# Gabrielcb/DaliID

Measured on AMD Instinct MI355X. Metric: images/sec (train step), higher is better.
Workload: dtype bf16; 1 GPU; configs[1]: ResNet-50 ReID bf16 256x128, PK batch 16x16=256 per GPU, center+proxy heads, Adam, EMA; global_batch=256, per_gpu_batch=256, parallelism=dp1

## Files before the change

daliid_amd/csrc/bnlin.hip:

```cpp
#include "kernels.h"
#include "reduce_finish.h"
#include <algorithm>

namespace dali {

namespace {
constexpr int BL_CH = 8;

__device__ __forceinline__ double block_sum_d(double v, double* red) {
    const int lane = threadIdx.x & 63, w = threadIdx.x >> 6;
#pragma unroll
    for (int o = 32; o > 0; o >>= 1) v += __shfl_xor(v, o, 64);
    __syncthreads();
    if (lane == 0) red[w] = v;
    __syncthreads();
    return (red[0] + red[1]) + (red[2] + red[3]);
}
__device__ __forceinline__ float ld_f(const float* p) { return *p; }
__device__ __forceinline__ float ld_f(const uint16_t* p) { return bf16_bits_to_f32(*p); }
}

constexpr int BL_SAV_MAX = 2048;
struct BnlinFin {
    const float* m2; double count; const float* gamma; const float* beta; float* running_mean; float* running_var; float momentum, eps;
// ... 359 lines not shown
    hipLaunchKernelGGL(bnlin_row_kernel, dim3(C / BL_CH), dim3(256), (size_t)(3 * BL_CH + 1) * w * sizeof(float), st, W, ut, m2, s_dz, C, w,
                       count, scale, mean, invstd, dW, dgamma, dbeta, wd1, ld1, qk);
    DALI_LAUNCH_CHECK();
#define BL_BWD(DEPTH) hipLaunchKernelGGL((bnlin_nt_gemm_kernel<uint16_t, true, true, false, DEPTH>), dim3(w / 32, w / 32), dim3(256), 0, st, Wt, C, Wt, C, qk, C, (float*)nullptr, wd2, ld2, \
                                         (const uint16_t*)nullptr, 0, (float*)nullptr, 0, qk + C, bvec)
    switch (C <= BL_SAV_MAX ? bnlin_depth(C) : 1) { case 8: BL_BWD(8); break; case 4: BL_BWD(4); break; case 2: BL_BWD(2); break; default: BL_BWD(1); }
#undef BL_BWD
    DALI_LAUNCH_CHECK();
    return DALI_OK;
}

}

using namespace dali;

static GatherGeom bl_geom(int P, int Ck) {
    GatherGeom g{};
    g.Hout = 1; g.Wout = P; g.Hin = 1; g.Win = P; g.Ck = Ck; g.R = 1; g.S = 1; g.stride = 1; g.pad = 0; g.mode = 0;
    g.pix_pitch = Ck; g.row_pitch = P * Ck; g.img_pitch = (long long)P * Ck; g.lw = g.lhw = -1;
    return g;
}

extern "C" int dali_bnlin_fwd(dali_ctx* ctx, void* stream, const uint16_t* a, const uint16_t* W, int P, int C, int w, const float* gamma,
                              const float* beta, float* running_mean, float* running_var, float momentum, float eps, float* gram, float* m2,
                              float* ut, float* scale, float* shift, float* mean, float* invstd) {
    DALI_REQUIRE(ctx && a && W && gamma && beta && gram && m2 && ut && scale && shift && mean && invstd, "dali_bnlin_fwd: null argument");
    DALI_REQUIRE(P > 0 && C % 32 == 0 && w % 32 == 0, "dali_bnlin_fwd: C %% 32, w %% 32 (C=%d w=%d)", C, w);
    hipStream_t st = (hipStream_t)stream;
    WGradArgs wa{};
    wa.dY = a; wa.X = a; wa.Cm = w; wa.P = P; wa.Ntot = w; wa.g = bl_geom(P, w);
    size_t wsb;
    wgrad_plan(w, w, P, 512, &wa.splits, &wa.pix_per_split, &wsb, 1, 0);
    const bool fused_cs = wgrad_colsum_supported(w, w, 1, P);
    const int cs_rows = wgrad_colsum_rows(w, w, 1, P, wa.splits);
    const size_t b_cs = align_up(std::max(colsum_partial_floats(P, w), (size_t)cs_rows * w) * 4, 256), b_sc = align_up(reduce_scratch_bytes(w, 1), 256);
    const size_t b_wt = align_up((size_t)C * w * 2, 256), b_dot = align_up((size_t)(w / 32) * C * 12, 256);
    char* ws = static_cast<char*>(workspace(ctx, align_up(wsb, 256) + b_cs + b_sc + b_wt + b_dot));
    if (!ws) return DALI_ERR_NOMEM;
    wa.partial = reinterpret_cast<float*>(ws);
    char* p = ws + align_up(wsb, 256);
    float* cs_partial = reinterpret_cast<float*>(p); p += b_cs;
    double* scratch = reinterpret_cast<double*>(p); p += b_sc;
    uint16_t* wt = reinterpret_cast<uint16_t*>(p); p += b_wt;
    float* dot = reinterpret_cast<float*>(p);
    int rc;
    if (fused_cs) wa.colsum = cs_partial;
    if ((rc = launch_igemm_wgrad(st, wa, gram, 0, fused_cs ? m2 : nullptr, cs_rows))) return rc;
    if (!fused_cs && (rc = launch_colsum(st, a, P, w, m2, cs_partial, scratch))) return rc;
    if ((rc = launch_weight_transpose(st, W, C, 1, w, wt))) return rc;
    return launch_bnlin_stats(st, W, wt, gram, m2, C, w, (double)P, gamma, beta, running_mean, running_var, momentum, eps, ut, dot, scale, shift, mean, invstd);
}

extern "C" int dali_bnlin_bwd(dali_ctx* ctx, void* stream, const uint16_t* dz, const uint16_t* a, const uint16_t* W, int P, int C, int w,
                              const float* ut, const float* m2, const float* scale, const float* mean, const float* invstd, float* dW,
                              float* dgamma, float* dbeta, uint16_t* wd1, uint16_t* wd2, float* bvec) {
    DALI_REQUIRE(ctx && dz && a && W && ut && m2 && scale && mean && invstd && dW && dgamma && dbeta && wd1 && wd2 && bvec, "dali_bnlin_bwd: null argument");
    DALI_REQUIRE(P > 0 && C % 32 == 0 && w % 32 == 0, "dali_bnlin_bwd: C %% 32, w %% 32 (C=%d w=%d)", C, w);
    hipStream_t st = (hipStream_t)stream;
    WGradArgs wa{};
    wa.dY = dz; wa.X = a; wa.Cm = C; wa.P = P; wa.Ntot = w; wa.g = bl_geom(P, w);
    size_t wsb;
    wgrad_plan(C, w, P, 512, &wa.splits, &wa.pix_per_split, &wsb, 1, 0);
    const bool fused_cs = wgrad_colsum_supported(C, w, 1, P);
    const int cs_rows = wgrad_colsum_rows(C, w, 1, P, wa.splits);
    const size_t b_cs = align_up(std::max(colsum_partial_floats(P, C), (size_t)cs_rows * C) * 4, 256), b_sc = align_up(reduce_scratch_bytes(C, 1), 256);
    const size_t b_v = align_up((size_t)C * 4, 256), b_wt = align_up((size_t)C * w * 2, 256);
    char* ws = static_cast<char*>(workspace(ctx, align_up(wsb, 256) + b_cs + b_sc + 3 * b_v + b_wt));
    if (!ws) return DALI_ERR_NOMEM;
    wa.partial = reinterpret_cast<float*>(ws);
    char* p = ws + align_up(wsb, 256);
    float* cs_partial = reinterpret_cast<float*>(p); p += b_cs;
    double* scratch = reinterpret_cast<double*>(p); p += b_sc;
    float* sdz = reinterpret_cast<float*>(p); p += b_v;
    float* qk = reinterpret_cast<float*>(p); p += 2 * b_v;
    uint16_t* wt = reinterpret_cast<uint16_t*>(p);
// ... 8 lines not shown
```

daliid_amd/csrc/conv.hip:

```cpp
#include "gemm_tile.h"
#include "kernels.h"
#include <cstdlib>
#include <type_traits>
#include <vector>
#include <string>
#include <cstdio>

namespace dali {

__device__ __forceinline__ void decode_pixel(const GatherGeom& g, int p, int& n, int& ho, int& wo) {
    if (g.lhw >= 0 && g.lw >= 0) {
        n = p >> g.lhw;
        const int rem = p & ((1 << g.lhw) - 1);
        ho = rem >> g.lw;
        wo = rem & ((1 << g.lw) - 1);
    } else {
        const int hw = g.Hout * g.Wout;
        n = p / hw;
        const int rem = p - n * hw;
        ho = rem / g.Wout;
        wo = rem - ho * g.Wout;
    }
}

// ... 1295 lines not shown
                const bf16x8_t fb = *reinterpret_cast<const bf16x8_t*>(patch + (boff[j] ^ (uint32_t)(h << 5)));
#pragma unroll
                for (int i = 0; i < FM; ++i) acc[i][j] = __builtin_amdgcn_mfma_f32_16x16x32_bf16(fa[i], fb, acc[i][j], 0, 0, 0);
            }
        }
        asm volatile("s_waitcnt lgkmcnt(0)" ::: "memory");
        __builtin_amdgcn_s_barrier();
    }
    conv_epilogue_g<TM, TN, FM, FN, 4, NT, (EPI == 3 || EPI == 5) ? EPI : 2>(a, acc, 0, tn, smem, 0, wn);
}

}
#include "fused1x1.h"
namespace dali {

__device__ __forceinline__ int wg_swz(int row) { return (row & 3) | (((row >> 3) & 1) << 2); }

typedef short s16x4_t __attribute__((ext_vector_type(4)));

__device__ __forceinline__ bf16x8_t tr_frag(const uint16_t* tile, int chunk32, int lane) {
    const int g = lane >> 4, q = (lane & 15) >> 2, p = lane & 3;
    const int row0 = 8 * g + q, row1 = row0 + 4;
    const int off0 = row0 * 128 + ((chunk32 ^ wg_swz(row0)) << 4) + 4 * p;
    const int off1 = row1 * 128 + ((chunk32 ^ wg_swz(row1)) << 4) + 4 * p;
    typedef __attribute__((address_space(3))) s16x4_t* lds_ptr_t;
    const s16x4_t a = __builtin_amdgcn_ds_read_tr16_b64_v4i16((lds_ptr_t)(tile + off0));
    const s16x4_t b = __builtin_amdgcn_ds_read_tr16_b64_v4i16((lds_ptr_t)(tile + off1));
    typedef short s16x8_t __attribute__((ext_vector_type(8)));
    const s16x8_t v = {a[0], a[1], a[2], a[3], b[0], b[1], b[2], b[3]};
    return __builtin_bit_cast(bf16x8_t, v);
}

struct TrPair { s16x4_t lo, hi; };
__device__ __forceinline__ s16x4_t ds_read_tr_raw(const uint16_t* p) {
    typedef __attribute__((address_space(3))) const uint16_t* lds_cptr_t;
    const uint32_t addr = (uint32_t)(uintptr_t)(lds_cptr_t)p;
    s16x4_t v;
    asm volatile("ds_read_b64_tr_b16 %0, %1" : "=v"(v) : "v"(addr));
    return v;
}
__device__ __forceinline__ TrPair tr_frag_raw(const uint16_t* tile, int chunk32, int lane) {
    const int g = lane >> 4, q = (lane & 15) >> 2, p = lane & 3;
    const int row0 = 8 * g + q, row1 = row0 + 4;
    const int off0 = row0 * 128 + ((chunk32 ^ wg_swz(row0)) << 4) + 4 * p;
    const int off1 = row1 * 128 + ((chunk32 ^ wg_swz(row1)) << 4) + 4 * p;
    return TrPair{ds_read_tr_raw(tile + off0), ds_read_tr_raw(tile + off1)};
}
__device__ __forceinline__ bf16x8_t tr_join(const TrPair& t) {
    typedef short s16x8_t __attribute__((ext_vector_type(8)));
    const s16x8_t v = {t.lo[0], t.lo[1], t.lo[2], t.lo[3], t.hi[0], t.hi[1], t.hi[2], t.hi[3]};
    return __builtin_bit_cast(bf16x8_t, v);
}
template <int N>
__device__ __forceinline__ void tr_settle(TrPair& a, TrPair& b, TrPair& c, TrPair& d) {
    static_assert(N == 0 || N == 8 || N == 10 || N == 16 || N == 18, "lgkmcnt immediates used by the callers");
    if constexpr (N == 0) asm volatile("s_waitcnt lgkmcnt(0)" : "+v"(a.lo), "+v"(a.hi), "+v"(b.lo), "+v"(b.hi), "+v"(c.lo), "+v"(c.hi), "+v"(d.lo), "+v"(d.hi));
    else if constexpr (N == 8) asm volatile("s_waitcnt lgkmcnt(8)" : "+v"(a.lo), "+v"(a.hi), "+v"(b.lo), "+v"(b.hi), "+v"(c.lo), "+v"(c.hi), "+v"(d.lo), "+v"(d.hi));
    else if constexpr (N == 10) asm volatile("s_waitcnt lgkmcnt(10)" : "+v"(a.lo), "+v"(a.hi), "+v"(b.lo), "+v"(b.hi), "+v"(c.lo), "+v"(c.hi), "+v"(d.lo), "+v"(d.hi));
    else if constexpr (N == 16) asm volatile("s_waitcnt lgkmcnt(15)" : "+v"(a.lo), "+v"(a.hi), "+v"(b.lo), "+v"(b.hi), "+v"(c.lo), "+v"(c.hi), "+v"(d.lo), "+v"(d.hi));
    else asm volatile("s_waitcnt lgkmcnt(15)" : "+v"(a.lo), "+v"(a.hi), "+v"(b.lo), "+v"(b.hi), "+v"(c.lo), "+v"(c.hi), "+v"(d.lo), "+v"(d.hi));
}

__device__ __forceinline__ void tr_settle_all(TrPair& a) { asm volatile("s_waitcnt lgkmcnt(0)" : "+v"(a.lo), "+v"(a.hi)); }

template <int FM, int FN>
__device__ __forceinline__ void store_slab_tiles(float* slab, const f32x4_t (&acc)[FM][FN], int m_first, int n_first, int Cm, int Ntot, int lane) {
    const int mr = m_first + (lane >> 4) * 4, nc = n_first + (lane & 15);
    if (m_first + 16 * FM <= Cm && n_first + 16 * FN <= Ntot) {
        float* row = slab + (size_t)mr * Ntot + nc;
#pragma unroll
        for (int i = 0; i < FM; ++i)
#pragma unroll
            for (int rr = 0; rr < 4; ++rr) {
                float* p = row + (size_t)(i * 16 + rr) * Ntot;
#pragma unroll
                for (int j = 0; j < FN; ++j) p[j * 16] = acc[i][j][rr];
            }
        return;
    }
#pragma unroll
    for (int i = 0; i < FM; ++i)
#pragma unroll
        for (int j = 0; j < FN; ++j) {
            const int n = nc + j * 16;
#pragma unroll
            for (int rr = 0; rr < 4; ++rr) {
                const int m = mr + i * 16 + rr;
                if (m < Cm && n < Ntot) slab[(size_t)m * Ntot + n] = acc[i][j][rr];
            }
        }
}

template <bool IN_BN>
__global__ __launch_bounds__(256) void igemm_wgrad_kernel(WGradArgs a, int tiles_m, int tiles_n) {
    constexpr int TILE = 32 * 128;
    __shared__ __attribute__((aligned(16))) uint16_t smem[2 * 2 * TILE];
    const int tid = threadIdx.x, lane = tid & 63, wave = tid >> 6;
    const int wm = wave >> 1, wn = wave & 1;
    const int tiles = tiles_m * tiles_n;
    const int tile = blockIdx.x % tiles, ks = blockIdx.x / tiles;
    const int tm = tile / tiles_n, tn = tile - tm * tiles_n;
    const int m0 = tm * 128, n0 = tn * 128;
    const GatherGeom g = a.g;

    const int c16 = tid & 15;
    const int am = m0 + c16 * 8;
// ... 1530 lines not shown
```

daliid_amd/csrc/kernels.h:

```cpp
#pragma once
#include "common.h"

namespace dali {

struct GatherGeom {
    int Hout, Wout;
    int Hin, Win;
    int Ck;
    int R, S, stride, pad;
    int mode;
    long long img_pitch;
    int row_pitch, pix_pitch;
    int lw, lhw;
    int sub, oph, opw, Hfull, Wfull;
    int r0, rstep, nr, s0, sstep, ns;
    int class_grid;
};

struct IGemmArgs {
    const uint16_t* W;
    const uint16_t* X;
    uint16_t* O;
    const uint16_t* Res;
    const uint8_t* res_mask;
// ... 45 lines not shown
void wgrad_plan(int Cm, int Ntot, int P, int target_blocks, int* splits, int* pix_per_split, size_t* ws_bytes, int taps = 1, int halo_w = 0);
int launch_igemm_wgrad(hipStream_t st, const WGradArgs& a, float* out, int accumulate, float* colsum_out = nullptr, int colsum_rows = 0);
int launch_splitk_reduce2(hipStream_t st, const float* partial, float* out, size_t elems, int splits, int accumulate,
                          const float* partial2, float* out2, size_t elems2, int splits2);
bool wgrad_colsum_supported(int Cm, int Ntot, int taps, int P);
int launch_splitk_reduce(hipStream_t st, const float* partial, float* out, size_t elems, int splits, int accumulate);

int launch_linear_fwd(hipStream_t st, const uint16_t* x, const uint16_t* w, const float* bias, int act, const uint16_t* residual, uint16_t* y,
                      uint16_t* pre, const uint16_t* dact_pre, int rows, int K, int N, const float* row_scale = nullptr);
int launch_linear_wgrad(hipStream_t st, const uint16_t* x, const uint16_t* dy, float* dw, int rows, int K, int N, float* slab,
                        float* dbias = nullptr, float* cs_partial = nullptr, bool* bias_done = nullptr);
size_t linear_wgrad_colsum_floats(int rows, int K, int N);
int wgrad_colsum_rows(int Cm, int Ntot, int taps, int P, int splits);
size_t linear_wgrad_slab_bytes(int rows, int K, int N);

int launch_bnlin_stats(hipStream_t st, const uint16_t* W, const uint16_t* Wt, const float* gram, const float* m2, int C, int w, double count, const float* gamma,
                       const float* beta, float* rm, float* rv, float momentum, float eps, float* ut, float* dot, float* scale, float* shift,
                       float* mean, float* invstd);
int launch_bnlin_ut(hipStream_t st, const uint16_t* W, const float* gram, int C, int w, float* ut);
int launch_bnlin_bwd(hipStream_t st, const uint16_t* W, const uint16_t* Wt, const float* ut, const float* m2, const float* s_dz, int C,
                     int w, double count, const float* scale, const float* mean, const float* invstd, float* dW, float* dgamma, float* dbeta,
                     uint16_t* wd1, uint16_t* wd2, float* bvec, float* qk, int ld1 = 0, int ld2 = 0);

constexpr int REDUCE_SMAX = 64;
inline size_t reduce_scratch_bytes(int C, int NV) { return (size_t)REDUCE_SMAX * C * NV * sizeof(double); }
int launch_bn_finalize(hipStream_t st, const float* partial, int tiles, int C, double count, const float* gamma, const float* beta,
                       float* rm, float* rv, float momentum, float eps, float* scale, float* shift, float* mean, float* invstd,
                       double* scratch);
int launch_bn_eval_coeffs(hipStream_t st, const float* gamma, const float* beta, const float* rm, const float* rv, float eps, int C,
                          float* scale, float* shift);
// ... 64 lines not shown
```

daliid_amd/csrc/resnet_plan.hip:

```cpp
#include "kernels.h"
#include <cstdio>
#include <cstring>
#include <new>
#include <string>
#include <vector>

using namespace dali;

namespace {

struct TensorInfo { std::string name; int64_t offset, numel; int shape[4]; int ndim; };

struct Conv {
    int cin, cout, r, s, stride, pad, hin, win, hout, wout;
    int64_t w_off;
    uint16_t* w_bf16;
    uint16_t* wt_bf16;
};
struct Bn {
    int C;
    int64_t g_off, b_off;
    int64_t rm_off, rv_off;
    float *scale, *shift, *mean, *invstd, *coef;
};
// ... 190 lines not shown
        int sp, pps; size_t wsb;
        wgrad_plan(wb, 224, (int)N * net->stem_h * net->stem_w, 512, &sp, &pps, &wsb, 7);
        max_slab = wsb;
    }
    for (auto& b : net->blocks) {
        const size_t pin = N * b.hin * b.win, pout = N * b.hout * b.wout;
        reserve(net, a, b.raw1, pin * b.width * 2);
        reserve(net, a, b.a1, pin * b.width * 2);
        reserve(net, a, b.raw2, pout * b.width * 2);
        reserve(net, a, b.a2, pout * b.width * 2);
        reserve(net, a, b.gram, (size_t)b.width * b.width * 4); reserve(net, a, b.m2, (size_t)b.width * 4);
        reserve(net, a, b.sdz, (size_t)b.cout * 4); reserve(net, a, b.bvec, (size_t)b.width * 4); reserve(net, a, b.qk, (size_t)b.cout * 8);
        reserve(net, a, b.wd1, (size_t)b.width * (b.cout + b.width) * 2);
        reserve(net, a, b.ut, (size_t)b.width * b.cout * 4); reserve(net, a, b.dot, (size_t)(b.width / 32) * b.cout * 12);
        max_cs = std::max(max_cs, std::max(colsum_partial_floats((int)pout, b.cout), colsum_partial_floats((int)pout, b.width)) * 4);
        int sp, pps; size_t wsb;
        wgrad_plan(b.width, b.width, (int)pout, 512, &sp, &pps, &wsb, 1, 0);
        max_slab = std::max(max_slab, wsb);
        max_cs = std::max(max_cs, (size_t)wgrad_colsum_rows(b.width, b.width, 1, (int)pout, sp) * b.width * 4);
        wgrad_plan(b.cout, b.width, (int)pout, 512, &sp, &pps, &wsb, 1, 0);
        max_cs = std::max(max_cs, (size_t)wgrad_colsum_rows(b.cout, b.width, 1, (int)pout, sp) * b.cout * 4);
        reserve(net, a, b.y, pout * b.cout * 2);
        reserve(net, a, b.ybits, pout * b.cout / 8);
        if (b.has_ds) reserve(net, a, b.rawd, pout * b.cout * 2);
        if (b.lin_ds) {
            reserve(net, a, b.gram_d, (size_t)b.cin * b.cin * 4); reserve(net, a, b.m2_d, (size_t)b.cin * 4);
            reserve(net, a, b.ut_d, (size_t)b.cin * b.cout * 4); reserve(net, a, b.bvec_d, (size_t)b.cin * 4); reserve(net, a, b.qk_d, (size_t)b.cout * 8);
            reserve(net, a, b.wdd, (size_t)b.cin * (b.cout + b.cin) * 2);
            int sp, pps; size_t wsb;
            wgrad_plan(b.cin, b.cin, (int)pin, 512, &sp, &pps, &wsb, 1, 0);
            max_slab = std::max(max_slab, wsb);
            max_cs = std::max(max_cs, std::max(colsum_partial_floats((int)pin, b.cin), (size_t)wgrad_colsum_rows(b.cin, b.cin, 1, (int)pin, sp) * b.cin) * 4);
        }
        b.cat_eval = b.has_ds && b.cd.stride == 1 && conv_cat_act_supported(b.cout, b.width, b.cin, (int)pout, 2);
        if (b.cat_eval) { reserve(net, a, b.wcat, (size_t)b.cout * 2 * (b.width + b.cin) * 2); reserve(net, a, b.shcat, (size_t)b.cout * 4); }
        reserve_bn(net, a, b.b1); reserve_bn(net, a, b.b2); reserve_bn(net, a, b.b3);
        if (b.has_ds) reserve_bn(net, a, b.bd);
        Conv* cs[4] = {&b.c1, &b.c2, &b.c3, b.has_ds ? &b.cd : nullptr};
        for (Conv* c : cs) {
            if (!c) continue;
            reserve(net, a, c->wt_bf16, (size_t)c->cin * c->r * c->s * c->cout * 2);
            const int P = (int)N * c->hout * c->wout;
            max_stat = std::max(max_stat, (size_t)igemm_conv_stat_tiles(c->cout, P, c->r * c->s * c->cin) * c->cout * 2 * 4);
            int sp, pps; size_t wsb;
            wgrad_plan(c->cout, c->r * c->s * c->cin, P, 512, &sp, &pps, &wsb, c->r * c->s, conv_halo_w(*c));
            max_slab = std::max(max_slab, wsb);
            max_act = std::max(max_act, (size_t)P * c->cout * 2);
// ... 186 lines not shown
    const uint16_t* x = net->pool0;
    for (auto& b : net->blocks) {
        b.x = const_cast<uint16_t*>(x);
        const size_t e1 = (size_t)net->N * b.hin * b.win * b.width, e2 = (size_t)net->N * b.hout * b.wout * b.width;
        if (!tr) {
            if ((rc = conv_bn_relu_eval(net, st, b.c1, b.b1, x, b.a1))) return rc;
            if ((rc = conv_bn_relu_eval(net, st, b.c2, b.b2, b.a1, b.a2))) return rc;
        } else {
            if ((rc = conv_bn_fwd(net, st, b.c1, b.b1, x, nullptr, b.raw1, tr))) return rc;
            if ((rc = launch_bn_act(st, b.raw1, b.b1.scale, b.b1.shift, nullptr, nullptr, nullptr, nullptr, 1, e1, b.width, b.a1, nullptr))) return rc;
            if ((rc = conv_bn_fwd(net, st, b.c2, b.b2, b.a1, nullptr, b.raw2, tr))) return rc;
            if ((rc = launch_bn_act(st, b.raw2, b.b2.scale, b.b2.shift, nullptr, nullptr, nullptr, nullptr, 1, e2, b.width, b.a2, nullptr))) return rc;
        }
        const int Pout = net->N * b.hout * b.wout;
        if (tr) {
            const Conv sq = square_conv(b.c3);
            WGradArgs wa{};
            wa.dY = b.a2; wa.X = b.a2; wa.partial = net->wgrad_slab; wa.Cm = b.width; wa.P = Pout; wa.Ntot = b.width;
            wa.g = conv_geom(sq, 0);
            size_t wsb;
            wgrad_plan(wa.Cm, wa.Ntot, wa.P, 512, &wa.splits, &wa.pix_per_split, &wsb, 1, 0);
            const bool fused_cs = wgrad_colsum_supported(wa.Cm, wa.Ntot, 1, wa.P);
            if (fused_cs) wa.colsum = net->cs_partial;
            if ((rc = launch_igemm_wgrad(st, wa, b.gram, 0, fused_cs ? b.m2 : nullptr, fused_cs ? wgrad_colsum_rows(wa.Cm, wa.Ntot, 1, wa.P, wa.splits) : 0))) return rc;
            if (!fused_cs && (rc = launch_colsum(st, b.a2, Pout, b.width, b.m2, net->cs_partial, net->red_scratch))) return rc;
            if ((rc = launch_bnlin_stats(st, b.c3.w_bf16, b.c3.wt_bf16, b.gram, b.m2, b.cout, b.width, (double)Pout, net->P + b.b3.g_off, net->P + b.b3.b_off,
                                         net->B + b.b3.rm_off, net->B + b.b3.rv_off, 0.1f, 1e-5f, b.ut, b.dot, b.b3.scale, b.b3.shift, b.b3.mean,
                                         b.b3.invstd))) return rc;
        }
        if (!tr && b.cat_eval) {
            if ((rc = launch_fold_cat_weights(st, net->P + b.c3.w_off, net->P + b.cd.w_off, b.b3.scale, b.bd.scale, b.b3.shift, b.bd.shift, b.cout, b.width,
                                              b.cin, 2, b.wcat, b.shcat))) return rc;
            IGemmArgs ca{};
            ca.W = b.wcat; ca.X = b.a2; ca.X2 = x; ca.Ck1 = b.width; ca.x_rep = 2; ca.O = b.y; ca.out_shift = b.shcat; ca.out_relu = 1;
            ca.Cm = b.cout; ca.P = Pout;
            Conv cat = b.c3;
            cat.cin = 2 * (b.width + b.cin);
            ca.g = conv_geom(cat, 0);
            if ((rc = launch_igemm_conv(st, ca))) return rc;
            x = b.y;
            continue;
        }
        IGemmArgs a{};
        a.W = b.c3.w_bf16; a.X = b.a2; a.O = b.y; a.Res = x; a.out_scale = b.b3.scale; a.out_shift = b.b3.shift; a.out_relu = 1;
        if (b.has_ds) {
            if ((rc = conv_bn_fwd(net, st, b.cd, b.bd, x, nullptr, b.rawd, tr))) return rc;
            a.Res = b.rawd; a.res_scale = b.bd.scale; a.bias = b.bd.shift;
            if (b.lin_ds && tr) {
                Conv sq = b.cd;
                sq.cout = b.cd.cin;
                WGradArgs wa{};
                wa.dY = x; wa.X = x; wa.partial = net->wgrad_slab; wa.Cm = b.cin; wa.P = Pout; wa.Ntot = b.cin;
                wa.g = conv_geom(sq, 0);
                size_t wsb;
                wgrad_plan(wa.Cm, wa.Ntot, wa.P, 512, &wa.splits, &wa.pix_per_split, &wsb, 1, 0);
                const bool fused_cs = wgrad_colsum_supported(wa.Cm, wa.Ntot, 1, wa.P);
                if (fused_cs) wa.colsum = net->cs_partial;
                if ((rc = launch_igemm_wgrad(st, wa, b.gram_d, 0, fused_cs ? b.m2_d : nullptr, fused_cs ? wgrad_colsum_rows(wa.Cm, wa.Ntot, 1, wa.P, wa.splits) : 0))) return rc;
                if (!fused_cs && (rc = launch_colsum(st, x, Pout, b.cin, b.m2_d, net->cs_partial, net->red_scratch))) return rc;
                if ((rc = launch_bnlin_ut(st, b.cd.w_bf16, b.gram_d, b.cout, b.cin, b.ut_d))) return rc;
            }
        }
        a.bits_out = tr ? b.ybits : nullptr;
        a.Cm = b.cout; a.P = Pout; a.g = conv_geom(b.c3, 0);
        if ((rc = launch_igemm_conv(st, a))) return rc;
        x = b.y;
    }
    if ((rc = launch_head_pool_fwd(st, x, net->N, net->head_hw, net->feat_dim, net->feature_mode, net->feat, net->head_arg))) return rc;
    return launch_bn1d_fwd(st, net->feat, net->N, net->feat_dim, net->P + net->neck.g_off, net->P + net->neck.b_off, net->B + net->neck.rm_off,
                           net->B + net->neck.rv_off, tr ? 1 : 0, 0.1f, 1e-5f, emb, net->neck_mean, net->neck_invstd);
}

static int block_backward(dali_resnet* net, hipStream_t st, Block& b, const uint8_t* prev_bits) {
    int rc;
// ... 176 lines not shown
```

include/daliid_debug.h:

```cpp
#ifndef DALIID_DEBUG_H
#define DALIID_DEBUG_H

#ifdef __cplusplus
extern "C" {
#endif

int dali_debug_reload_env(void);

int dali_debug_set_conv_stamps(void* dev_ptr);

int dali_debug_wgrad_splits(int Cm, int Ntot, int P, int taps, int halo_w);

int dali_debug_splitk_reduce(void* stream, const float* partial, float* out, long long elems, int splits, int accumulate);

struct dali_resnet;
int dali_debug_resnet_backward_block(struct dali_resnet* net, void* stream, const float* d_emb, int block);

#ifdef __cplusplus
}
#endif
#endif
```

Before: 17450 images/s.

## Add dedicated streaming Gram kernel with fused column sums for BN-linear stats

```diff
diff --git a/daliid_amd/csrc/bnlin.hip b/daliid_amd/csrc/bnlin.hip
--- a/daliid_amd/csrc/bnlin.hip
+++ b/daliid_amd/csrc/bnlin.hip
@@ -397,39 +397,26 @@
 
 using namespace dali;
 
-static GatherGeom bl_geom(int P, int Ck) {
-    GatherGeom g{};
-    g.Hout = 1; g.Wout = P; g.Hin = 1; g.Win = P; g.Ck = Ck; g.R = 1; g.S = 1; g.stride = 1; g.pad = 0; g.mode = 0;
-    g.pix_pitch = Ck; g.row_pitch = P * Ck; g.img_pitch = (long long)P * Ck; g.lw = g.lhw = -1;
-    return g;
-}
-
 extern "C" int dali_bnlin_fwd(dali_ctx* ctx, void* stream, const uint16_t* a, const uint16_t* W, int P, int C, int w, const float* gamma,
                               const float* beta, float* running_mean, float* running_var, float momentum, float eps, float* gram, float* m2,
                               float* ut, float* scale, float* shift, float* mean, float* invstd) {
     DALI_REQUIRE(ctx && a && W && gamma && beta && gram && m2 && ut && scale && shift && mean && invstd, "dali_bnlin_fwd: null argument");
     DALI_REQUIRE(P > 0 && C % 32 == 0 && w % 32 == 0, "dali_bnlin_fwd: C %% 32, w %% 32 (C=%d w=%d)", C, w);
     hipStream_t st = (hipStream_t)stream;
-    WGradArgs wa{};
-    wa.dY = a; wa.X = a; wa.Cm = w; wa.P = P; wa.Ntot = w; wa.g = bl_geom(P, w);
-    size_t wsb;
-    wgrad_plan(w, w, P, 512, &wa.splits, &wa.pix_per_split, &wsb, 1, 0);
-    const bool fused_cs = wgrad_colsum_supported(w, w, 1, P);
-    const int cs_rows = wgrad_colsum_rows(w, w, 1, P, wa.splits);
-    const size_t b_cs = align_up(std::max(colsum_partial_floats(P, w), (size_t)cs_rows * w) * 4, 256), b_sc = align_up(reduce_scratch_bytes(w, 1), 256);
+    size_t wsb, csb;
+    gram_workspace_bytes(P, w, &wsb, &csb);
+    const size_t b_cs = align_up(csb, 256), b_sc = align_up(reduce_scratch_bytes(w, 1), 256);
     const size_t b_wt = align_up((size_t)C * w * 2, 256), b_dot = align_up((size_t)(w / 32) * C * 12, 256);
     char* ws = static_cast<char*>(workspace(ctx, align_up(wsb, 256) + b_cs + b_sc + b_wt + b_dot));
     if (!ws) return DALI_ERR_NOMEM;
-    wa.partial = reinterpret_cast<float*>(ws);
+    float* slab = reinterpret_cast<float*>(ws);
     char* p = ws + align_up(wsb, 256);
     float* cs_partial = reinterpret_cast<float*>(p); p += b_cs;
     double* scratch = reinterpret_cast<double*>(p); p += b_sc;
     uint16_t* wt = reinterpret_cast<uint16_t*>(p); p += b_wt;
     float* dot = reinterpret_cast<float*>(p);
     int rc;
-    if (fused_cs) wa.colsum = cs_partial;
-    if ((rc = launch_igemm_wgrad(st, wa, gram, 0, fused_cs ? m2 : nullptr, cs_rows))) return rc;
-    if (!fused_cs && (rc = launch_colsum(st, a, P, w, m2, cs_partial, scratch))) return rc;
+    if ((rc = launch_gram(st, a, P, w, plain_rows_geom(P, w), gram, m2, slab, cs_partial, scratch))) return rc;
     if ((rc = launch_weight_transpose(st, W, C, 1, w, wt))) return rc;
     return launch_bnlin_stats(st, W, wt, gram, m2, C, w, (double)P, gamma, beta, running_mean, running_var, momentum, eps, ut, dot, scale, shift, mean, invstd);
 }
@@ -441,7 +428,7 @@
     DALI_REQUIRE(P > 0 && C % 32 == 0 && w % 32 == 0, "dali_bnlin_bwd: C %% 32, w %% 32 (C=%d w=%d)", C, w);
     hipStream_t st = (hipStream_t)stream;
     WGradArgs wa{};
-    wa.dY = dz; wa.X = a; wa.Cm = C; wa.P = P; wa.Ntot = w; wa.g = bl_geom(P, w);
+    wa.dY = dz; wa.X = a; wa.Cm = C; wa.P = P; wa.Ntot = w; wa.g = plain_rows_geom(P, w);
     size_t wsb;
     wgrad_plan(C, w, P, 512, &wa.splits, &wa.pix_per_split, &wsb, 1, 0);
     const bool fused_cs = wgrad_colsum_supported(C, w, 1, P);
diff --git a/daliid_amd/csrc/conv.hip b/daliid_amd/csrc/conv.hip
--- a/daliid_amd/csrc/conv.hip
+++ b/daliid_amd/csrc/conv.hip
@@ -1,4 +1,5 @@
 #include "gemm_tile.h"
+#include "wgrad_frag.h"
 #include "kernels.h"
 #include <cstdlib>
 #include <type_traits>
@@ -1333,82 +1334,6 @@
 #include "fused1x1.h"
 namespace dali {
 
-__device__ __forceinline__ int wg_swz(int row) { return (row & 3) | (((row >> 3) & 1) << 2); }
-
-typedef short s16x4_t __attribute__((ext_vector_type(4)));
-
-__device__ __forceinline__ bf16x8_t tr_frag(const uint16_t* tile, int chunk32, int lane) {
-    const int g = lane >> 4, q = (lane & 15) >> 2, p = lane & 3;
-    const int row0 = 8 * g + q, row1 = row0 + 4;
-    const int off0 = row0 * 128 + ((chunk32 ^ wg_swz(row0)) << 4) + 4 * p;
-    const int off1 = row1 * 128 + ((chunk32 ^ wg_swz(row1)) << 4) + 4 * p;
-    typedef __attribute__((address_space(3))) s16x4_t* lds_ptr_t;
-    const s16x4_t a = __builtin_amdgcn_ds_read_tr16_b64_v4i16((lds_ptr_t)(tile + off0));
-    const s16x4_t b = __builtin_amdgcn_ds_read_tr16_b64_v4i16((lds_ptr_t)(tile + off1));
-    typedef short s16x8_t __attribute__((ext_vector_type(8)));
-    const s16x8_t v = {a[0], a[1], a[2], a[3], b[0], b[1], b[2], b[3]};
-    return __builtin_bit_cast(bf16x8_t, v);
-}
-
-struct TrPair { s16x4_t lo, hi; };
-__device__ __forceinline__ s16x4_t ds_read_tr_raw(const uint16_t* p) {
-    typedef __attribute__((address_space(3))) const uint16_t* lds_cptr_t;
-    const uint32_t addr = (uint32_t)(uintptr_t)(lds_cptr_t)p;
-    s16x4_t v;
-    asm volatile("ds_read_b64_tr_b16 %0, %1" : "=v"(v) : "v"(addr));
-    return v;
-}
-__device__ __forceinline__ TrPair tr_frag_raw(const uint16_t* tile, int chunk32, int lane) {
-    const int g = lane >> 4, q = (lane & 15) >> 2, p = lane & 3;
-    const int row0 = 8 * g + q, row1 = row0 + 4;
-    const int off0 = row0 * 128 + ((chunk32 ^ wg_swz(row0)) << 4) + 4 * p;
-    const int off1 = row1 * 128 + ((chunk32 ^ wg_swz(row1)) << 4) + 4 * p;
-    return TrPair{ds_read_tr_raw(tile + off0), ds_read_tr_raw(tile + off1)};
-}
-__device__ __forceinline__ bf16x8_t tr_join(const TrPair& t) {
-    typedef short s16x8_t __attribute__((ext_vector_type(8)));
-    const s16x8_t v = {t.lo[0], t.lo[1], t.lo[2], t.lo[3], t.hi[0], t.hi[1], t.hi[2], t.hi[3]};
-    return __builtin_bit_cast(bf16x8_t, v);
-}
-template <int N>
-__device__ __forceinline__ void tr_settle(TrPair& a, TrPair& b, TrPair& c, TrPair& d) {
-    static_assert(N == 0 || N == 8 || N == 10 || N == 16 || N == 18, "lgkmcnt immediates used by the callers");
-    if constexpr (N == 0) asm volatile("s_waitcnt lgkmcnt(0)" : "+v"(a.lo), "+v"(a.hi), "+v"(b.lo), "+v"(b.hi), "+v"(c.lo), "+v"(c.hi), "+v"(d.lo), "+v"(d.hi));
-    else if constexpr (N == 8) asm volatile("s_waitcnt lgkmcnt(8)" : "+v"(a.lo), "+v"(a.hi), "+v"(b.lo), "+v"(b.hi), "+v"(c.lo), "+v"(c.hi), "+v"(d.lo), "+v"(d.hi));
-    else if constexpr (N == 10) asm volatile("s_waitcnt lgkmcnt(10)" : "+v"(a.lo), "+v"(a.hi), "+v"(b.lo), "+v"(b.hi), "+v"(c.lo), "+v"(c.hi), "+v"(d.lo), "+v"(d.hi));
-    else if constexpr (N == 16) asm volatile("s_waitcnt lgkmcnt(15)" : "+v"(a.lo), "+v"(a.hi), "+v"(b.lo), "+v"(b.hi), "+v"(c.lo), "+v"(c.hi), "+v"(d.lo), "+v"(d.hi));
-    else asm volatile("s_waitcnt lgkmcnt(15)" : "+v"(a.lo), "+v"(a.hi), "+v"(b.lo), "+v"(b.hi), "+v"(c.lo), "+v"(c.hi), "+v"(d.lo), "+v"(d.hi));
-}
-
-__device__ __forceinline__ void tr_settle_all(TrPair& a) { asm volatile("s_waitcnt lgkmcnt(0)" : "+v"(a.lo), "+v"(a.hi)); }
-
-template <int FM, int FN>
-__device__ __forceinline__ void store_slab_tiles(float* slab, const f32x4_t (&acc)[FM][FN], int m_first, int n_first, int Cm, int Ntot, int lane) {
-    const int mr = m_first + (lane >> 4) * 4, nc = n_first + (lane & 15);
-    if (m_first + 16 * FM <= Cm && n_first + 16 * FN <= Ntot) {
-        float* row = slab + (size_t)mr * Ntot + nc;
-#pragma unroll
-        for (int i = 0; i < FM; ++i)
-#pragma unroll
-            for (int rr = 0; rr < 4; ++rr) {
-                float* p = row + (size_t)(i * 16 + rr) * Ntot;
-#pragma unroll
-                for (int j = 0; j < FN; ++j) p[j * 16] = acc[i][j][rr];
-            }
-        return;
-    }
-#pragma unroll
-    for (int i = 0; i < FM; ++i)
-#pragma unroll
-        for (int j = 0; j < FN; ++j) {
-            const int n = nc + j * 16;
-#pragma unroll
-            for (int rr = 0; rr < 4; ++rr) {
-                const int m = mr + i * 16 + rr;
-                if (m < Cm && n < Ntot) slab[(size_t)m * Ntot + n] = acc[i][j][rr];
-            }
-        }
-}
 
 template <bool IN_BN>
 __global__ __launch_bounds__(256) void igemm_wgrad_kernel(WGradArgs a, int tiles_m, int tiles_n) {
diff --git a/daliid_amd/csrc/gram.hip b/daliid_amd/csrc/gram.hip
--- /dev/null
+++ b/daliid_amd/csrc/gram.hip
@@ -0,0 +1,236 @@
+#include "gemm_tile.h"
+#include "wgrad_frag.h"
+#include "gram_plan.h"
+#include "kernels.h"
+#include <algorithm>
+#include <cstdio>
+
+namespace dali {
+
+struct GramArgs {
+    const uint16_t* a;
+    float* slab;
+    float* cs;
+    int P, ksteps, steps_per_range, wgs;
+};
+
+constexpr int GRAM_PANEL = 32 * 128;
+constexpr int gram_stages(int panels) { return panels == 1 ? 8 : 6; }
+constexpr int gram_lds_bytes(int w) { return w == 256 ? gram_stages(2) * 2 * GRAM_PANEL * 2 : gram_stages(1) * GRAM_PANEL * 2; }
+
+template <int N>
+__device__ __forceinline__ void gram_wait() {
+    static_assert(N >= 0 && N < 64, "vmcnt is a 6-bit count");
+    asm volatile("s_waitcnt vmcnt(%0) lgkmcnt(0)" ::"n"(N) : "memory");
+}
+
+template <int W, int NP>
+__device__ __forceinline__ void gram_block(const GramArgs& g, uint16_t* smem, int range, int bi, int bj) {
+    constexpr int D = gram_stages(NP), PPW = 2 * NP;
+    constexpr int KP = W == 64 ? 64 : 32, ROW = W == 64 ? 128 : W;
+    const int tid = threadIdx.x, lane = tid & 63;
+    const int wave = __builtin_amdgcn_readfirstlane(tid >> 6);
+    const int w_hi = wave >> 1, w_lo = wave & 1;
+    const __amdgpu_buffer_rsrc_t rs = __builtin_amdgcn_make_buffer_rsrc(const_cast<uint16_t*>(g.a), 0, g.P * W * 2, 0x00020000);
+
+    const int r_in = lane >> 4, ps = lane & 15;
+    const int c16 = ((((ps >> 1) ^ wg_swz(4 * wave + r_in)) << 1) | (ps & 1));
+    const uint32_t lane_off = (uint32_t)((4 * wave + r_in) * ROW + c16 * 8);
+    const uint32_t col[2] = {W == 64 ? 0u : (uint32_t)bi * 128u, W == 64 ? 0u : (uint32_t)bj * 128u};
+
+    const int k0 = range * g.steps_per_range;
+    const int nk = min(g.steps_per_range, g.ksteps - k0);
+
+    auto issue = [&](int kt, int stage) {
+        const uint32_t base = (uint32_t)(k0 + kt) * (uint32_t)(KP * W) + lane_off;
+#pragma unroll
+        for (int q = 0; q < NP; ++q)
+#pragma unroll
+            for (int i = 0; i < 2; ++i) {
+                const uint32_t off = kt < nk ? (base + col[q] + (uint32_t)(i * 16 * ROW)) * 2u : DMA_OOB;
+                __builtin_amdgcn_raw_ptr_buffer_load_lds(rs, (lds_void_ptr)(smem + (stage * NP + q) * GRAM_PANEL + (wave + 4 * i) * 512), 16, off, 0, 0, 0);
+            }
+    };
+
+    constexpr int FN = W == 64 ? 2 : 4;
+    const int ca = w_hi * 4;
+    const int cb = W == 64 ? w_hi * 4 + w_lo * 2 : w_lo * 4;
+    f32x4_t acc[4][FN], cs[4];
+#pragma unroll
+    for (int i = 0; i < 4; ++i) {
+        cs[i] = f32x4_t{0.f, 0.f, 0.f, 0.f};
+#pragma unroll
+        for (int j = 0; j < FN; ++j) acc[i][j] = f32x4_t{0.f, 0.f, 0.f, 0.f};
+    }
+    const bool do_cs = w_lo == 0 && bj == 0;
+    typedef short ones_vec_t __attribute__((ext_vector_type(8)));
+    const bf16x8_t ones = __builtin_bit_cast(bf16x8_t, ones_vec_t{0x3F80, 0x3F80, 0x3F80, 0x3F80, 0x3F80, 0x3F80, 0x3F80, 0x3F80});
+
+#pragma unroll
+    for (int s = 0; s < D - 1; ++s) issue(s, s);
+    gram_wait<(D - 2) * PPW>();
+    __builtin_amdgcn_s_barrier();
+    int st_cur = 0, st_nxt = D - 1;
+    for (int kt = 0; kt < nk; ++kt) {
+        issue(kt + D - 1, st_nxt);
+        const uint16_t* sa = smem + st_cur * NP * GRAM_PANEL;
+        const uint16_t* sb = sa + (NP - 1) * GRAM_PANEL;
+        TrPair ra[4], rb[FN];
+#pragma unroll
+        for (int i = 0; i < 4; ++i) ra[i] = tr_frag_raw(sa, ca + i, lane);
+#pragma unroll
+        for (int j = 0; j < FN; ++j) rb[j] = tr_frag_raw(sb, cb + j, lane);
+        if constexpr (FN == 4) {
+            tr_settle<8>(ra[0], ra[1], ra[2], ra[3]);
+            tr_settle<0>(rb[0], rb[1], rb[2], rb[3]);
+        } else {
+            tr_settle<0>(ra[0], ra[1], ra[2], ra[3]);
+            tr_settle_all(rb[0]);
+            tr_settle_all(rb[1]);
+        }
+        bf16x8_t fa[4];
+#pragma unroll
+        for (int i = 0; i < 4; ++i) fa[i] = tr_join(ra[i]);
+#pragma unroll
+        for (int j = 0; j < FN; ++j) {
+            const bf16x8_t fb = tr_join(rb[j]);
+#pragma unroll
+            for (int i = 0; i < 4; ++i) acc[i][j] = __builtin_amdgcn_mfma_f32_16x16x32_bf16(fa[i], fb, acc[i][j], 0, 0, 0);
+        }
+        if (do_cs) {
+#pragma unroll
+            for (int i = 0; i < 4; ++i) cs[i] = __builtin_amdgcn_mfma_f32_16x16x32_bf16(fa[i], ones, cs[i], 0, 0, 0);
+        }
+        gram_wait<(D - 2) * PPW>();
+        __builtin_amdgcn_s_barrier();
+        st_cur = (st_cur == D - 1) ? 0 : st_cur + 1;
+        st_nxt = (st_nxt == D - 1) ? 0 : st_nxt + 1;
+    }
+    gram_wait<0>();
+
+    float* slab = g.slab + (size_t)range * W * W;
+    float* csrow = g.cs + (size_t)range * W;
+    if constexpr (W == 64) {
+        __builtin_amdgcn_s_barrier();
+        float* x = reinterpret_cast<float*>(smem) + (w_lo * 48) * 64 + lane;
+        if (w_hi == 1) {
+#pragma unroll
+            for (int i = 0; i < 4; ++i)
+#pragma unroll
+                for (int rr = 0; rr < 4; ++rr) {
+#pragma unroll
+                    for (int j = 0; j < 2; ++j) x[((i * 2 + j) * 4 + rr) * 64] = acc[i][j][rr];
+                    x[(32 + i * 4 + rr) * 64] = cs[i][rr];
+                }
+        }
+        __syncthreads();
+        if (w_hi == 0) {
+#pragma unroll
+            for (int i = 0; i < 4; ++i)
+#pragma unroll
+                for (int rr = 0; rr < 4; ++rr) {
+#pragma unroll
+                    for (int j = 0; j < 2; ++j) acc[i][j][rr] += x[((i * 2 + j) * 4 + rr) * 64];
+                    cs[i][rr] += x[(32 + i * 4 + rr) * 64];
+                }
+            store_slab_tiles<4, 2>(slab, acc, 0, w_lo * 32, 64, 64, lane);
+            if (do_cs && (lane & 15) == 0) {
+#pragma unroll
+                for (int i = 0; i < 4; ++i)
+#pragma unroll
+                    for (int rr = 0; rr < 4; ++rr) csrow[i * 16 + (lane >> 4) * 4 + rr] = cs[i][rr];
+            }
+        }
+    } else {
+        store_slab_tiles<4, 4>(slab, acc, bi * 128 + w_hi * 64, bj * 128 + w_lo * 64, W, W, lane);
+        if (do_cs && (lane & 15) == 0) {
+#pragma unroll
+            for (int i = 0; i < 4; ++i)
+#pragma unroll
+                for (int rr = 0; rr < 4; ++rr) csrow[bi * 128 + w_hi * 64 + i * 16 + (lane >> 4) * 4 + rr] = cs[i][rr];
+        }
+    }
+}
+
+template <int W>
+__global__ __launch_bounds__(256) void gram_stream_kernel(GramArgs g) {
+    extern __shared__ __attribute__((aligned(16))) uint16_t smem[];
+    constexpr int BLOCKS = W == 256 ? 4 : 1;
+    const int per = (g.wgs + 7) >> 3;
+    const int item = (blockIdx.x & 7) * per + (blockIdx.x >> 3);
+    if (item >= g.wgs) return;
+    const int range = item / BLOCKS, blk = item - range * BLOCKS;
+    if constexpr (W == 256) {
+        const int bi = blk >> 1, bj = blk & 1;
+        if (bi == bj) gram_block<W, 1>(g, smem, range, bi, bj);
+        else gram_block<W, 2>(g, smem, range, bi, bj);
+    } else {
+        gram_block<W, 1>(g, smem, range, 0, 0);
+    }
+}
+
+GatherGeom plain_rows_geom(int P, int Ck) {
+    GatherGeom g{};
+    g.Hout = 1; g.Wout = P; g.Hin = 1; g.Win = P; g.Ck = Ck; g.R = 1; g.S = 1; g.stride = 1; g.pad = 0; g.mode = 0;
+    g.pix_pitch = Ck; g.row_pitch = P * Ck; g.img_pitch = (long long)P * Ck; g.lw = g.lhw = -1;
+    return g;
+}
+
+void gram_workspace_bytes(int P, int w, size_t* slab_bytes, size_t* cs_bytes) {
+    int sp, pps; size_t wsb;
+    wgrad_plan(w, w, P, 512, &sp, &pps, &wsb, 1, 0);
+    const size_t cs = std::max(colsum_partial_floats(P, w), (size_t)wgrad_colsum_rows(w, w, 1, P, sp) * w) * sizeof(float);
+    gram_cover_bytes(P, w, wsb, cs, slab_bytes, cs_bytes);
+}
+
+int launch_gram_colsum(hipStream_t st, const uint16_t* a, int P, int w, float* gram_out, float* m2_out, float* slab, float* cs_partial) {
+    if (!gram_stream_supported(P, w)) { set_error("gram: the streaming kernel takes w = 64, 128, 256 and tensors below 2 GiB (P=%d w=%d)", P, w); return DALI_ERR_UNSUPPORTED; }
+    const GramPlan p = gram_plan(P, w);
+    GramArgs g{a, slab, cs_partial, P, p.ksteps, p.steps_per_range, p.wgs};
+    const int lds = gram_lds_bytes(w), grid = (p.wgs + 7) / 8 * 8;
+    {
+        char what[160] = "";
+        snprintf(what, sizeof what, "wgrad,Cm=%d,K=%d,P=%d,taps=1,stride=1,sub=0,fused=0,stats=0,res=0,mask=0,lin=1,gram=1", w, w, P);
+        const int slot = gemm_profile_begin(st, 1, 2.0 * (double)P * w * w, what);
+#define GRAM_LAUNCH(W_)                                                                                                                                  \
+    do {                                                                                                                                                 \
+        DALI_ONCE_PER_DEVICE(DALI_HIP(hipFuncSetAttribute(reinterpret_cast<const void*>(&gram_stream_kernel<W_>), hipFuncAttributeMaxDynamicSharedMemorySize, lds))); \
+        hipLaunchKernelGGL(gram_stream_kernel<W_>, dim3(grid), dim3(256), lds, st, g);                                                                    \
+    } while (0)
+        if (w == 64) GRAM_LAUNCH(64); else if (w == 128) GRAM_LAUNCH(128); else GRAM_LAUNCH(256);
+#undef GRAM_LAUNCH
+        gemm_profile_end(st, slot);
+        DALI_LAUNCH_CHECK();
+    }
+    return launch_splitk_reduce2(st, slab, gram_out, (size_t)w * w, p.ranges, 0, cs_partial, m2_out, (size_t)w, p.ranges);
+}
+
+int launch_gram(hipStream_t st, const uint16_t* a, int P, int w, const GatherGeom& geom, float* gram_out, float* m2_out, float* slab, float* cs_partial,
+                double* scratch, int path) {
+    if (path == 2 || (path == 0 && gram_use_stream(P, w))) return launch_gram_colsum(st, a, P, w, gram_out, m2_out, slab, cs_partial);
+    WGradArgs wa{};
+    wa.dY = a; wa.X = a; wa.partial = slab; wa.Cm = w; wa.P = P; wa.Ntot = w; wa.g = geom;
+    size_t wsb;
+    wgrad_plan(w, w, P, 512, &wa.splits, &wa.pix_per_split, &wsb, 1, 0);
+    const bool fused_cs = wgrad_colsum_supported(w, w, 1, P);
+    if (fused_cs) wa.colsum = cs_partial;
+    if (int rc = launch_igemm_wgrad(st, wa, gram_out, 0, fused_cs ? m2_out : nullptr, fused_cs ? wgrad_colsum_rows(w, w, 1, P, wa.splits) : 0)) return rc;
+    if (!fused_cs) return launch_colsum(st, a, P, w, m2_out, cs_partial, scratch);
+    return DALI_OK;
+}
+
+}
+
+using namespace dali;
+
+extern "C" int dali_debug_gram(dali_ctx* ctx, void* stream, const uint16_t* a, int P, int w, float* gram, float* m2, int path) {
+    DALI_REQUIRE(ctx && a && gram && m2, "dali_debug_gram: null argument");
+    DALI_REQUIRE(P > 0 && w > 0 && w % 32 == 0 && path >= 0 && path <= 2, "dali_debug_gram: P > 0, w %% 32, path 0..2 (P=%d w=%d path=%d)", P, w, path);
+    size_t b_slab, b_cs;
+    gram_workspace_bytes(P, w, &b_slab, &b_cs);
+    b_slab = align_up(b_slab, 256); b_cs = align_up(b_cs, 256);
+    char* ws = static_cast<char*>(workspace(ctx, b_slab + b_cs + align_up(reduce_scratch_bytes(w, 1), 256)));
+    if (!ws) return DALI_ERR_NOMEM;
+    return launch_gram(static_cast<hipStream_t>(stream), a, P, w, plain_rows_geom(P, w), gram, m2, reinterpret_cast<float*>(ws), reinterpret_cast<float*>(ws + b_slab),
+                       reinterpret_cast<double*>(ws + b_slab + b_cs), path);
+}
diff --git a/daliid_amd/csrc/gram_plan.h b/daliid_amd/csrc/gram_plan.h
--- /dev/null
+++ b/daliid_amd/csrc/gram_plan.h
@@ -0,0 +1,49 @@
+#pragma once
+#include <stddef.h>
+
+namespace dali {
+
+constexpr int GRAM_MIN_STEPS = 8;
+
+struct GramPlan {
+    int kp;
+    int ksteps;
+    int steps_per_range;
+    int ranges;
+    int blocks;
+    int wgs;
+    size_t slab_bytes;
+    size_t cs_bytes;
+};
+
+inline bool gram_stream_supported(long long P, int w) {
+    return (w == 64 || w == 128 || w == 256) && P > 0 && P * w * 2 <= (1ll << 31) - (1ll << 16);
+}
+
+inline GramPlan gram_plan(int P, int w) {
+    GramPlan g{};
+    g.kp = w == 64 ? 64 : 32;
+    g.ksteps = (P + g.kp - 1) / g.kp;
+    g.blocks = w == 256 ? 4 : 1;
+    const int max_ranges = 256 / g.blocks;
+    int spr = (g.ksteps + max_ranges - 1) / max_ranges;
+    if (spr < GRAM_MIN_STEPS) spr = GRAM_MIN_STEPS;
+    g.steps_per_range = spr;
+    g.ranges = (g.ksteps + spr - 1) / spr;
+    g.wgs = g.ranges * g.blocks;
+    g.slab_bytes = (size_t)g.ranges * w * w * sizeof(float);
+    g.cs_bytes = (size_t)g.ranges * w * sizeof(float);
+    return g;
+}
+
+inline void gram_cover_bytes(int P, int w, size_t gemm_slab_bytes, size_t gemm_cs_bytes, size_t* slab_bytes, size_t* cs_bytes) {
+    *slab_bytes = gemm_slab_bytes; *cs_bytes = gemm_cs_bytes;
+    if (!gram_stream_supported(P, w)) return;
+    const GramPlan g = gram_plan(P, w);
+    if (g.slab_bytes > *slab_bytes) *slab_bytes = g.slab_bytes;
+    if (g.cs_bytes > *cs_bytes) *cs_bytes = g.cs_bytes;
+}
+
+inline bool gram_use_stream(long long P, int w) { return gram_stream_supported(P, w); }
+
+}
diff --git a/daliid_amd/csrc/kernels.h b/daliid_amd/csrc/kernels.h
--- a/daliid_amd/csrc/kernels.h
+++ b/daliid_amd/csrc/kernels.h
@@ -83,6 +83,12 @@
 int wgrad_colsum_rows(int Cm, int Ntot, int taps, int P, int splits);
 size_t linear_wgrad_slab_bytes(int rows, int K, int N);
 
+GatherGeom plain_rows_geom(int P, int Ck);
+void gram_workspace_bytes(int P, int w, size_t* slab_bytes, size_t* cs_bytes);
+int launch_gram_colsum(hipStream_t st, const uint16_t* a, int P, int w, float* gram_out, float* m2_out, float* slab, float* cs_partial);
+int launch_gram(hipStream_t st, const uint16_t* a, int P, int w, const GatherGeom& geom, float* gram_out, float* m2_out, float* slab, float* cs_partial,
+                double* scratch, int path = 0);
+
 int launch_bnlin_stats(hipStream_t st, const uint16_t* W, const uint16_t* Wt, const float* gram, const float* m2, int C, int w, double count, const float* gamma,
                        const float* beta, float* rm, float* rv, float momentum, float eps, float* ut, float* dot, float* scale, float* shift,
                        float* mean, float* invstd);
diff --git a/daliid_amd/csrc/resnet_plan.hip b/daliid_amd/csrc/resnet_plan.hip
--- a/daliid_amd/csrc/resnet_plan.hip
+++ b/daliid_amd/csrc/resnet_plan.hip
@@ -228,10 +228,10 @@
         reserve(net, a, b.wd1, (size_t)b.width * (b.cout + b.width) * 2);
         reserve(net, a, b.ut, (size_t)b.width * b.cout * 4); reserve(net, a, b.dot, (size_t)(b.width / 32) * b.cout * 12);
         max_cs = std::max(max_cs, std::max(colsum_partial_floats((int)pout, b.cout), colsum_partial_floats((int)pout, b.width)) * 4);
-        int sp, pps; size_t wsb;
-        wgrad_plan(b.width, b.width, (int)pout, 512, &sp, &pps, &wsb, 1, 0);
+        int sp, pps; size_t wsb, csb;
+        gram_workspace_bytes((int)pout, b.width, &wsb, &csb);
         max_slab = std::max(max_slab, wsb);
-        max_cs = std::max(max_cs, (size_t)wgrad_colsum_rows(b.width, b.width, 1, (int)pout, sp) * b.width * 4);
+        max_cs = std::max(max_cs, csb);
         wgrad_plan(b.cout, b.width, (int)pout, 512, &sp, &pps, &wsb, 1, 0);
         max_cs = std::max(max_cs, (size_t)wgrad_colsum_rows(b.cout, b.width, 1, (int)pout, sp) * b.cout * 4);
         reserve(net, a, b.y, pout * b.cout * 2);
@@ -241,10 +241,10 @@
             reserve(net, a, b.gram_d, (size_t)b.cin * b.cin * 4); reserve(net, a, b.m2_d, (size_t)b.cin * 4);
             reserve(net, a, b.ut_d, (size_t)b.cin * b.cout * 4); reserve(net, a, b.bvec_d, (size_t)b.cin * 4); reserve(net, a, b.qk_d, (size_t)b.cout * 8);
             reserve(net, a, b.wdd, (size_t)b.cin * (b.cout + b.cin) * 2);
-            int sp, pps; size_t wsb;
-            wgrad_plan(b.cin, b.cin, (int)pin, 512, &sp, &pps, &wsb, 1, 0);
+            size_t wsb, csb;
+            gram_workspace_bytes((int)pin, b.cin, &wsb, &csb);
             max_slab = std::max(max_slab, wsb);
-            max_cs = std::max(max_cs, std::max(colsum_partial_floats((int)pin, b.cin), (size_t)wgrad_colsum_rows(b.cin, b.cin, 1, (int)pin, sp) * b.cin) * 4);
+            max_cs = std::max(max_cs, csb);
         }
         b.cat_eval = b.has_ds && b.cd.stride == 1 && conv_cat_act_supported(b.cout, b.width, b.cin, (int)pout, 2);
         if (b.cat_eval) { reserve(net, a, b.wcat, (size_t)b.cout * 2 * (b.width + b.cin) * 2); reserve(net, a, b.shcat, (size_t)b.cout * 4); }
@@ -461,16 +461,7 @@
         }
         const int Pout = net->N * b.hout * b.wout;
         if (tr) {
-            const Conv sq = square_conv(b.c3);
-            WGradArgs wa{};
-            wa.dY = b.a2; wa.X = b.a2; wa.partial = net->wgrad_slab; wa.Cm = b.width; wa.P = Pout; wa.Ntot = b.width;
-            wa.g = conv_geom(sq, 0);
-            size_t wsb;
-            wgrad_plan(wa.Cm, wa.Ntot, wa.P, 512, &wa.splits, &wa.pix_per_split, &wsb, 1, 0);
-            const bool fused_cs = wgrad_colsum_supported(wa.Cm, wa.Ntot, 1, wa.P);
-            if (fused_cs) wa.colsum = net->cs_partial;
-            if ((rc = launch_igemm_wgrad(st, wa, b.gram, 0, fused_cs ? b.m2 : nullptr, fused_cs ? wgrad_colsum_rows(wa.Cm, wa.Ntot, 1, wa.P, wa.splits) : 0))) return rc;
-            if (!fused_cs && (rc = launch_colsum(st, b.a2, Pout, b.width, b.m2, net->cs_partial, net->red_scratch))) return rc;
+            if ((rc = launch_gram(st, b.a2, Pout, b.width, conv_geom(square_conv(b.c3), 0), b.gram, b.m2, net->wgrad_slab, net->cs_partial, net->red_scratch))) return rc;
             if ((rc = launch_bnlin_stats(st, b.c3.w_bf16, b.c3.wt_bf16, b.gram, b.m2, b.cout, b.width, (double)Pout, net->P + b.b3.g_off, net->P + b.b3.b_off,
                                          net->B + b.b3.rm_off, net->B + b.b3.rv_off, 0.1f, 1e-5f, b.ut, b.dot, b.b3.scale, b.b3.shift, b.b3.mean,
                                          b.b3.invstd))) return rc;
@@ -496,15 +487,7 @@
             if (b.lin_ds && tr) {
                 Conv sq = b.cd;
                 sq.cout = b.cd.cin;
-                WGradArgs wa{};
-                wa.dY = x; wa.X = x; wa.partial = net->wgrad_slab; wa.Cm = b.cin; wa.P = Pout; wa.Ntot = b.cin;
-                wa.g = conv_geom(sq, 0);
-                size_t wsb;
-                wgrad_plan(wa.Cm, wa.Ntot, wa.P, 512, &wa.splits, &wa.pix_per_split, &wsb, 1, 0);
-                const bool fused_cs = wgrad_colsum_supported(wa.Cm, wa.Ntot, 1, wa.P);
-                if (fused_cs) wa.colsum = net->cs_partial;
-                if ((rc = launch_igemm_wgrad(st, wa, b.gram_d, 0, fused_cs ? b.m2_d : nullptr, fused_cs ? wgrad_colsum_rows(wa.Cm, wa.Ntot, 1, wa.P, wa.splits) : 0))) return rc;
-                if (!fused_cs && (rc = launch_colsum(st, x, Pout, b.cin, b.m2_d, net->cs_partial, net->red_scratch))) return rc;
+                if ((rc = launch_gram(st, x, Pout, b.cin, conv_geom(sq, 0), b.gram_d, b.m2_d, net->wgrad_slab, net->cs_partial, net->red_scratch))) return rc;
                 if ((rc = launch_bnlin_ut(st, b.cd.w_bf16, b.gram_d, b.cout, b.cin, b.ut_d))) return rc;
             }
         }
diff --git a/daliid_amd/csrc/wgrad_frag.h b/daliid_amd/csrc/wgrad_frag.h
--- /dev/null
+++ b/daliid_amd/csrc/wgrad_frag.h
@@ -0,0 +1,83 @@
+#pragma once
+#include "common.h"
+
+namespace dali {
+
+__device__ __forceinline__ int wg_swz(int row) { return (row & 3) | (((row >> 3) & 1) << 2); }
+
+typedef short s16x4_t __attribute__((ext_vector_type(4)));
+
+__device__ __forceinline__ bf16x8_t tr_frag(const uint16_t* tile, int chunk32, int lane) {
+    const int g = lane >> 4, q = (lane & 15) >> 2, p = lane & 3;
+    const int row0 = 8 * g + q, row1 = row0 + 4;
+    const int off0 = row0 * 128 + ((chunk32 ^ wg_swz(row0)) << 4) + 4 * p;
+    const int off1 = row1 * 128 + ((chunk32 ^ wg_swz(row1)) << 4) + 4 * p;
+    typedef __attribute__((address_space(3))) s16x4_t* lds_ptr_t;
+    const s16x4_t a = __builtin_amdgcn_ds_read_tr16_b64_v4i16((lds_ptr_t)(tile + off0));
+    const s16x4_t b = __builtin_amdgcn_ds_read_tr16_b64_v4i16((lds_ptr_t)(tile + off1));
+    typedef short s16x8_t __attribute__((ext_vector_type(8)));
+    const s16x8_t v = {a[0], a[1], a[2], a[3], b[0], b[1], b[2], b[3]};
+    return __builtin_bit_cast(bf16x8_t, v);
+}
+
+struct TrPair { s16x4_t lo, hi; };
+__device__ __forceinline__ s16x4_t ds_read_tr_raw(const uint16_t* p) {
+    typedef __attribute__((address_space(3))) const uint16_t* lds_cptr_t;
+    const uint32_t addr = (uint32_t)(uintptr_t)(lds_cptr_t)p;
+    s16x4_t v;
+    asm volatile("ds_read_b64_tr_b16 %0, %1" : "=v"(v) : "v"(addr));
+    return v;
+}
+__device__ __forceinline__ TrPair tr_frag_raw(const uint16_t* tile, int chunk32, int lane) {
+    const int g = lane >> 4, q = (lane & 15) >> 2, p = lane & 3;
+    const int row0 = 8 * g + q, row1 = row0 + 4;
+    const int off0 = row0 * 128 + ((chunk32 ^ wg_swz(row0)) << 4) + 4 * p;
+    const int off1 = row1 * 128 + ((chunk32 ^ wg_swz(row1)) << 4) + 4 * p;
+    return TrPair{ds_read_tr_raw(tile + off0), ds_read_tr_raw(tile + off1)};
+}
+__device__ __forceinline__ bf16x8_t tr_join(const TrPair& t) {
+    typedef short s16x8_t __attribute__((ext_vector_type(8)));
+    const s16x8_t v = {t.lo[0], t.lo[1], t.lo[2], t.lo[3], t.hi[0], t.hi[1], t.hi[2], t.hi[3]};
+    return __builtin_bit_cast(bf16x8_t, v);
+}
+template <int N>
+__device__ __forceinline__ void tr_settle(TrPair& a, TrPair& b, TrPair& c, TrPair& d) {
+    static_assert(N == 0 || N == 8 || N == 10 || N == 16 || N == 18, "lgkmcnt immediates used by the callers");
+    if constexpr (N == 0) asm volatile("s_waitcnt lgkmcnt(0)" : "+v"(a.lo), "+v"(a.hi), "+v"(b.lo), "+v"(b.hi), "+v"(c.lo), "+v"(c.hi), "+v"(d.lo), "+v"(d.hi));
+    else if constexpr (N == 8) asm volatile("s_waitcnt lgkmcnt(8)" : "+v"(a.lo), "+v"(a.hi), "+v"(b.lo), "+v"(b.hi), "+v"(c.lo), "+v"(c.hi), "+v"(d.lo), "+v"(d.hi));
+    else if constexpr (N == 10) asm volatile("s_waitcnt lgkmcnt(10)" : "+v"(a.lo), "+v"(a.hi), "+v"(b.lo), "+v"(b.hi), "+v"(c.lo), "+v"(c.hi), "+v"(d.lo), "+v"(d.hi));
+    else if constexpr (N == 16) asm volatile("s_waitcnt lgkmcnt(15)" : "+v"(a.lo), "+v"(a.hi), "+v"(b.lo), "+v"(b.hi), "+v"(c.lo), "+v"(c.hi), "+v"(d.lo), "+v"(d.hi));
+    else asm volatile("s_waitcnt lgkmcnt(15)" : "+v"(a.lo), "+v"(a.hi), "+v"(b.lo), "+v"(b.hi), "+v"(c.lo), "+v"(c.hi), "+v"(d.lo), "+v"(d.hi));
+}
+
+__device__ __forceinline__ void tr_settle_all(TrPair& a) { asm volatile("s_waitcnt lgkmcnt(0)" : "+v"(a.lo), "+v"(a.hi)); }
+
+template <int FM, int FN>
+__device__ __forceinline__ void store_slab_tiles(float* slab, const f32x4_t (&acc)[FM][FN], int m_first, int n_first, int Cm, int Ntot, int lane) {
+    const int mr = m_first + (lane >> 4) * 4, nc = n_first + (lane & 15);
+    if (m_first + 16 * FM <= Cm && n_first + 16 * FN <= Ntot) {
+        float* row = slab + (size_t)mr * Ntot + nc;
+#pragma unroll
+        for (int i = 0; i < FM; ++i)
+#pragma unroll
+            for (int rr = 0; rr < 4; ++rr) {
+                float* p = row + (size_t)(i * 16 + rr) * Ntot;
+#pragma unroll
+                for (int j = 0; j < FN; ++j) p[j * 16] = acc[i][j][rr];
+            }
+        return;
+    }
+#pragma unroll
+    for (int i = 0; i < FM; ++i)
+#pragma unroll
+        for (int j = 0; j < FN; ++j) {
+            const int n = nc + j * 16;
+#pragma unroll
+            for (int rr = 0; rr < 4; ++rr) {
+                const int m = mr + i * 16 + rr;
+                if (m < Cm && n < Ntot) slab[(size_t)m * Ntot + n] = acc[i][j][rr];
+            }
+        }
+}
+
+}
diff --git a/include/daliid_debug.h b/include/daliid_debug.h
--- a/include/daliid_debug.h
+++ b/include/daliid_debug.h
@@ -1,5 +1,6 @@
 #ifndef DALIID_DEBUG_H
 #define DALIID_DEBUG_H
+#include <stdint.h>
 
 #ifdef __cplusplus
 extern "C" {
@@ -13,6 +14,9 @@
 
 int dali_debug_splitk_reduce(void* stream, const float* partial, float* out, long long elems, int splits, int accumulate);
 
+struct dali_ctx;
+int dali_debug_gram(struct dali_ctx* ctx, void* stream, const uint16_t* a, int P, int w, float* gram, float* m2, int path);
+
 struct dali_resnet;
 int dali_debug_resnet_backward_block(struct dali_resnet* net, void* stream, const float* d_emb, int block);
 
```

New measurement: 17600 images/s, median of 6. About the same (+0.9%).
